# cherise215/advchain

Measured on AMD Instinct MI355X. Metric: augmented images/sec (N adv steps, chain=noise+bias+morph+affine), higher is better.
Workload: dtype f32

## Files before the change

advchain_amd/_lib.py:

```python
import ctypes
import os
from ctypes import c_char_p, c_float, c_int, c_int64, c_void_p

_HERE = os.path.dirname(os.path.abspath(__file__))
LIB_PATH = os.path.join(_HERE, "csrc", "libadvchain_hip.so")

_P, _I, _L, _F = c_void_p, c_int, c_int64, c_float

PROTOTYPES = {
    "advchain_version": (_I, []),
    "advchain_last_error": (c_char_p, []),
    "advchain_set_deterministic": (None, [_I]),
    "advchain_get_deterministic": (_I, []),
    "advchain_grid_sample_fwd": (_I, [_P, _P, _P, _L, _L, _I, _P, _P, _I, _I, _I, _P]),
    "advchain_grid_sample_fwd_ride": (_I, [_P, _P, _P, _P, _P, _L, _L, _I, _P, _P, _I, _I, _I, _I, _P]),
    "advchain_scatter_workspace": (_L, [_L, _I, _P]),
    "advchain_grid_sample_bwd": (_I, [_P, _P, _P, _P, _P, _P, _L, _L, _I, _P, _P, _I, _I, _I, _I, _P]),
    "advchain_compose_self_fwd": (_I, [_P, _P, _P, _L, _I, _P, _I, _P, _P]),
    "advchain_compose_self_bwd": (_I, [_P, _P, _P, _P, _I, _I, _L, _I, _P, _P]),
    "advchain_affine_warp_fwd": (_I, [_P, _P, _P, _L, _L, _I, _P, _I, _I, _P]),
    "advchain_affine_warp_fwd_ride": (_I, [_P, _P, _P, _P, _P, _L, _L, _I, _P, _I, _I, _I, _P]),
    "advchain_affine_warp_bwd_workspace": (_L, [_L, _I, _P]),
    "advchain_affine_warp_bwd": (_I, [_P, _P, _P, _P, _P, _P, _L, _L, _I, _P, _I, _I, _P]),
    "advchain_affine_theta_fwd": (_I, [_P, _P, _F, _P, _P, _L, _I, _P]),
    "advchain_affine_theta_bwd": (_I, [_P, _P, _F, _P, _P, _P, _L, _I, _P]),
    "advchain_tp_interp_fwd": (_I, [_P, _P, _P, _P, _P, _P, _P, _L, _L, _I, _I, _F, _P, _P, _P]),
    "advchain_tp_interp_fwd_smoothed_pair": (_I, [_P, _P, _P, _P, _P, _P, _P, _P, _L, _L, _I, _F, _P, _P, _F, _P]),
    "advchain_band_reduce_axis": (_I, [_P, _P, _P, _P, _P, _P, _P, _P, _I, _L, _L, _F, _P]),
    "advchain_band_reduce_rows_dense": (_I, [_P, _P, _P, _P, _P, _L, _L, _L, _L, _F, _P]),
    "advchain_bias_field_fwd": (_I, [_P, _P, _P, _P, _P, _P, _P, _P, _P, _L, _L, _F, _I, _F, _P]),
    "advchain_bias_field_bwd": (_I, [_P, _P, _P, _P, _P, _P, _P, _P, _P, _P, _L, _L, _F, _I, _F, _P]),
    "advchain_gauss_axis": (_I, [_P, _P, _P, _L, _L, _I, _P, _I, _P, _I, _I, _F, _P]),
    "advchain_gauss_axis_generic": (_I, [_P, _P, _L, _I, _P, _I, _P, _I, _F, _P]),
    "advchain_max_displacement": (_I, [_P, _P, _L, _I, _P, _P]),
    "advchain_grid_sample_bicubic2d_fwd": (_I, [_P, _P, _P, _L, _L, _P, _P, _I, _P]),
    "advchain_grid_sample_bicubic2d_bwd": (_I, [_P, _P, _P, _P, _P, _L, _L, _P, _P, _I, _P]),
    "advchain_affine_grid2d_fwd": (_I, [_P, _P, _L, _P, _P]),
    "advchain_affine_grid2d_bwd_workspace": (_L, [_L, _P]),
    "advchain_affine_grid2d_bwd": (_I, [_P, _P, _P, _L, _P, _P]),
    "advchain_slot_rows_max": (_I, [_P, _P, _L, _L, _I, _P]),
    "advchain_demons_compose_pair_fwd": (_I, [_P, _P, _P, _P, _P, _P, _P, _P, _P, _P, _P, _P, _P, _L, _I, _I, _P, _P, _F, _F, _I, _P]),
    "advchain_demons_compose_pair_bwd": (_I, [_P, _P, _P, _P, _P, _P, _P, _P, _P, _P, _P, _P, _P, _P, _P, _P, _P, _L, _P, _P, _P, _L,
                                              _I, _I, _P, _F, _F, _P]),
    "advchain_bounds_check": (_I, [_P, _P, _P, _L, _P, _P]),
    "advchain_expo_chain_fused_levels": (_I, [_L, _I, _P, _I, _P]),
    "advchain_expo_chain_fwd": (_I, [_P, _P, _P, _L, _I, _P, _I, _P, _P, _P, _P]),
    "advchain_expo_chain_bwd": (_I, [_P, _P, _P, _P, _P, _P, _P, _L, _I, _P, _I, _P]),
    "advchain_gauss_xy": (_I, [_P, _P, _P, _L, _L, _I, _P, _P, _I, _I, _F, _P, _P, _L]),
    "advchain_gauss_small": (_I, [_P, _P, _L, _I, _P, _P, _I, _F, _P]),
    "advchain_gauss_small_pair": (_I, [_P, _P, _L, _I, _P, _P, _F, _I, _P]),
    "advchain_axpy": (_I, [_P, _P, _P, _F, _L, _P]),
    "advchain_sign_axpy": (_I, [_P, _P, _P, _F, _L, _P, _P, _P]),
    "advchain_nonzero_mask": (_I, [_P, _P, _L, _P]),
    "advchain_consistency_finish": (_I, [_P, _P, _P, _P, _I, _P]),
    "advchain_norm_workspace": (_L, [_L, _L]),
    "advchain_norm_axpy": (_I, [_P, _P, _P, _P, _F, _L, _L, _P]),
    "advchain_norm_axpy_gated": (_I, [_P, _P, _P, _P, _F, _L, _L, _P, _P, _P]),
    "advchain_update_multi": (_I, [_P, _I, _P, _P]),
    "advchain_consistency_fwd": (_I, [_P, _P, _P, _P, _P, _P, _P, _L, _L, _I, _P, _I, _I, _I, _I, _P]),
    "advchain_consistency_bwd": (_I, [_P, _P, _P, _P, _P, _P, _F, _F, _F, _F, _I, _L, _L, _I, _P, _I, _P]),
    "advchain_consistency_fused_fwd": (_I, [_P, _P, _P, _P, _P, _L, _L, _I, _P, _I, _I, _I, _I, _P]),
    "advchain_consistency_fused_bwd": (_I, [_P, _P, _P, _P, _P, _P, _F, _F, _F, _F, _I, _L, _L, _I, _P, _I, _P]),
    "advchain_consistency_wide_fwd": (_I, [_P, _P, _P, _P, _P, _P, _L, _L, _I, _P, _I, _I, _I, _I, _P]),
    "advchain_consistency_wide_bwd": (_I, [_P, _P, _P, _P, _P, _P, _P, _F, _F, _F, _F, _I, _L, _L, _I, _P, _I, _P]),
    "advchain_consistency_fused_fwd_bf16": (_I, [_P, _P, _P, _P, _P, _L, _L, _I, _P, _P]),
    "advchain_consistency_fused_bwd_bf16": (_I, [_P, _P, _P, _P, _P, _P, _F, _F, _F, _L, _L, _I, _P, _P]),
# ... 112 lines not shown
```

advchain_amd/csrc/error.cpp:

```cpp
#include <string.h>

#include <atomic>

static thread_local char g_last_error[512] = "";

extern "C" void advchain_set_error_(const char* msg) {
  strncpy(g_last_error, msg ? msg : "", sizeof(g_last_error) - 1);
  g_last_error[sizeof(g_last_error) - 1] = 0;
}

extern "C" const char* advchain_last_error(void) { return g_last_error; }

static std::atomic<int> g_deterministic{0};
extern "C" void advchain_set_deterministic(int on) { g_deterministic.store(on ? 1 : 0, std::memory_order_relaxed); }
extern "C" int advchain_get_deterministic(void) { return g_deterministic.load(std::memory_order_relaxed); }

extern "C" int advchain_version(void) { return 130; }
```

advchain_amd/csrc/sampler_common.h:

```cpp
#pragma once
#include "common.h"

namespace advchain {

template <int DIM, int PAD>
struct Taps {
  AxisTap x, y, z;
  __device__ __forceinline__ void build(float gx, float gy, float gz, const Dims& d) {
    x = make_tap<PAD>(gx, d.s2);
    y = make_tap<PAD>(gy, d.s1);
    if (DIM == 3) z = make_tap<PAD>(gz, d.s0);
    else { z.i0 = 0; z.w0 = 1.f; z.w1 = 0.f; z.mult = 0.f; z.v0 = true; z.v1 = false; }
  }
  __device__ __forceinline__ bool ok(int cz, int cy, int cx) const {
    return (cx ? x.v1 : x.v0) && (cy ? y.v1 : y.v0) && (DIM == 3 ? (cz ? z.v1 : z.v0) : true);
  }
  __device__ __forceinline__ int off(int cz, int cy, int cx, const Dims& d) const {
    return ((z.i0 + cz) * d.s1 + (y.i0 + cy)) * d.s2 + (x.i0 + cx);
  }
  __device__ __forceinline__ float wx(int c) const { return c ? x.w1 : x.w0; }
  __device__ __forceinline__ float wy(int c) const { return c ? y.w1 : y.w0; }
  __device__ __forceinline__ float wz(int c) const { return c ? z.w1 : z.w0; }
  __device__ __forceinline__ float w(int cz, int cy, int cx) const {
    float r = wx(cx) * wy(cy);
// ... 134 lines not shown
  bx = affine_base_coord(ix, d.s2);
  by = affine_base_coord(iy, d.s1);
  if constexpr (DIM == 3) {
    bz = affine_base_coord(iz, d.s0);
    gx = th.m[0][0] * bx + th.m[0][1] * by + th.m[0][2] * bz + th.m[0][3];
    gy = th.m[1][0] * bx + th.m[1][1] * by + th.m[1][2] * bz + th.m[1][3];
    gz = th.m[DIM - 1][0] * bx + th.m[DIM - 1][1] * by + th.m[DIM - 1][2] * bz + th.m[DIM - 1][DIM];
  } else {
    bz = 0.f; gz = 0.f;
    gx = th.m[0][0] * bx + th.m[0][1] * by + th.m[0][2];
    gy = th.m[1][0] * bx + th.m[1][1] * by + th.m[1][2];
  }
}

template <int VEC>
__device__ __forceinline__ void load_vec(const float* __restrict__ p, float (&r)[VEC]) {
  if constexpr (VEC == 4) {
    const float4 q = *reinterpret_cast<const float4*>(p);
    r[0] = q.x; r[1] = q.y; r[2] = q.z; r[3] = q.w;
  } else {
#pragma unroll
    for (int k = 0; k < VEC; ++k) r[k] = p[k];
  }
}
template <int VEC>
__device__ __forceinline__ void store_vec(float* __restrict__ p, const float (&r)[VEC]) {
  if constexpr (VEC == 4) {
    *reinterpret_cast<float4*>(p) = make_float4(r[0], r[1], r[2], r[3]);
  } else {
#pragma unroll
    for (int k = 0; k < VEC; ++k) p[k] = r[k];
  }
}

__device__ __forceinline__ void lds_order() { asm volatile("" ::: "memory"); }

__device__ __forceinline__ float clamp_unit(float v) { return fminf(fmaxf(v, -1.f), 1.f); }

__device__ __forceinline__ float voxel_displacement(float g, int S, int s) {
  const float dv = fabsf(((g + 1.f) * 0.5f) * (float)(S - 1) - (float)s);
  return dv < 1.0e9f ? dv : 1.0e9f;
}

constexpr int kDispSlots = 4096;
__device__ __forceinline__ void wave_max_to_slots(float m, float* __restrict__ slots) {
#pragma unroll
  for (int o = 32; o > 0; o >>= 1) m = fmaxf(m, __shfl_xor(m, o, 64));
  const unsigned blk = (blockIdx.z * gridDim.y + blockIdx.y) * gridDim.x + blockIdx.x;
  float* p = slots + (blk * (blockDim.x >> 6) + (threadIdx.x >> 6)) % kDispSlots;
  if ((threadIdx.x & 63) == __builtin_ffsll(__builtin_amdgcn_ballot_w64(true)) - 1 && m > 0.f)
    atomicMax(reinterpret_cast<unsigned int*>(p), __float_as_uint(m));
}


}
```

advchain_amd/csrc/scatter_tiled.hip:

```cpp
#include <stdlib.h>
#include "sampler_common.h"

namespace advchain {

struct TileCfg {
  int t0, t1, t2;
  int h0, h1, h2;
  int n0, n1, n2;
};

__device__ __forceinline__ bool in_tile_box(int s, int u, int T, int H) {
  const int lo = (u / T) * T;
  return (s >= lo - H) && (s < lo + T + H);
}

__device__ __forceinline__ bool deposit_handled(int sz, int sy, int sx, int uz, int uy, int ux, const TileCfg& tc) {
  return in_tile_box(sx, ux, tc.t2, tc.h2) && in_tile_box(sy, uy, tc.t1, tc.h1) && in_tile_box(sz, uz, tc.t0, tc.h0);
}

constexpr int kFixedBits = 30;

__device__ __forceinline__ void lds_add_fixed(long long* p, float v) {
  const long long q = (long long)__float2int_rn(v);
  atomicAdd(reinterpret_cast<unsigned long long*>(p), (unsigned long long)q);
// ... 317 lines not shown
  }
}

int advchain_scatter_tiled_launch(bool self, const float* gout, const float* in, const float* grid, float* gin,
                                  float* ggrid, int64_t N, int64_t C, int ndim, Dims d, int padding, int clamp_grid,
                                  int32_t* workspace, int chain, int halo, hipStream_t st) {
  if (C < 1 || C > 4) return ADVCHAIN_ERR_UNSUPPORTED;
  const TileCfg tc = choose_tiles(ndim, d, (int)C, halo < 0 ? -halo : halo);
  const int64_t V = d.voxels();
  int* cnt = workspace;
  float* amax = reinterpret_cast<float*>(workspace + 2);
  int2* list = reinterpret_cast<int2*>(workspace + 4);
  const int64_t cap64 = N * V;
  const int cap = cap64 > 0x7fffffff ? 0x7fffffff : (int)cap64;
  hipLaunchKernelGGL(k_scatter_prepare, dim3(1), dim3(1), 0, st, workspace, chain);
  {
    const int64_t total = N * C * V;
    int blocks = (int)((total / 4 + kBlock - 1) / kBlock);
    if (blocks > 1024) blocks = 1024;
    if (blocks < 1) blocks = 1;
    hipLaunchKernelGGL(k_absmax, dim3(blocks), dim3(kBlock), 0, st, gout, total, amax,
                       (int)((reinterpret_cast<uintptr_t>(gout) & 15) == 0), chain ? workspace + 1 : (const int*)nullptr);
  }
  dim3 g((unsigned)(tc.n0 * tc.n1 * tc.n2), (unsigned)N);
  const size_t lds = (size_t)C * tc.t0 * tc.t1 * tc.t2 * sizeof(long long);
  const bool need_ggrid = ggrid != nullptr;
  bool ok;
#define GO(DIM_, PAD_) \
  ok = launch_rows_c<DIM_, PAD_>((int)C, self, need_ggrid, g, lds, st, gout, in, grid, gin, ggrid, d, tc, clamp_grid, amax, amax + 1, cnt, list, cap)
  if (ndim == 3) {
    switch (padding) {
      case PAD_ZEROS: GO(3, PAD_ZEROS); break;
      case PAD_BORDER: GO(3, PAD_BORDER); break;
      default: GO(3, PAD_REFLECTION); break;
    }
  } else {
    switch (padding) {
      case PAD_ZEROS: GO(2, PAD_ZEROS); break;
      case PAD_BORDER: GO(2, PAD_BORDER); break;
      default: GO(2, PAD_REFLECTION); break;
    }
  }
#undef GO
  if (!ok) return ADVCHAIN_ERR_UNSUPPORTED;
  ADVCHAIN_LAUNCH_CHECK();
  return ADVCHAIN_OK;
}

extern "C" int advchain_get_deterministic(void);
extern "C" int64_t advchain_scatter_workspace(int64_t N, int ndim, const int64_t* dims) {
  int64_t V = 1;
  for (int i = 0; i < ndim; ++i) V *= dims[i];
  const int64_t base = 4 + 2 * N * V;
  return advchain_get_deterministic() ? base + 8 * N * V + ((N + 3) & ~(int64_t)3) : base;
}
```

advchain_amd/csrc/scatter_window.hip:

```cpp
#include <stdlib.h>
#include "sampler_common.h"

namespace advchain {

constexpr int kDetBits = 40;
template <bool DET>
__device__ __forceinline__ void win_global_add(float* __restrict__ gin, unsigned long long* __restrict__ acc, int64_t idx,
                                               float v, const FixScale& sdet) {
  if (DET) atomicAdd(acc + idx, (unsigned long long)__float2ll_rn(fix_in(v * sdet.mul, sdet)));
  else atomic_add_f32(gin + idx, v);
}
__device__ __forceinline__ FixScale det_scale(const float* __restrict__ maxn, int n) { return fix_scale(maxn[n], kDetBits); }

__global__ void __launch_bounds__(kBlock) k_det_absmax(const float* __restrict__ x, float* __restrict__ maxn, int64_t per_n) {
  const int n = blockIdx.y;
  const float* p = x + (int64_t)n * per_n;
  float m = 0.f;
  bool bad = false;
  const int64_t stride = (int64_t)gridDim.x * kBlock * 4;
  for (int64_t i = ((int64_t)blockIdx.x * kBlock + threadIdx.x) * 4; i < per_n; i += stride) {
    float v[4];
    if (i + 4 <= per_n && ((uintptr_t)(p + i) & 15) == 0) {
      const float4 q = *reinterpret_cast<const float4*>(p + i);
      v[0] = q.x; v[1] = q.y; v[2] = q.z; v[3] = q.w;
    } else {
#pragma unroll
      for (int j = 0; j < 4; ++j) v[j] = i + j < per_n ? p[i + j] : 0.f;
    }
#pragma unroll
    for (int j = 0; j < 4; ++j) { m = fmaxf(m, fabsf(v[j])); bad = bad || !(fabsf(v[j]) <= 3.0e38f); }
  }
  if (bad) m = __int_as_float(0x7f800000);
#pragma unroll
  for (int o = 32; o > 0; o >>= 1) m = fmaxf(m, __shfl_xor(m, o, 64));
  __shared__ float wm[kBlock / 64];
  if ((threadIdx.x & 63) == 0) wm[threadIdx.x >> 6] = m;
  __syncthreads();
  if (threadIdx.x == 0) {
#pragma unroll
    for (int w = 1; w < kBlock / 64; ++w) m = fmaxf(m, wm[w]);
    atomicMax(reinterpret_cast<int*>(maxn) + n, __float_as_int(m));
  }
}

__global__ void __launch_bounds__(kBlock) k_det_convert(const long long* __restrict__ acc, const float* __restrict__ maxn,
                                                        float* __restrict__ gin, int64_t per_n) {
  const int n = blockIdx.y;
  const FixScale fs = det_scale(maxn, n);
  const long long* a = acc + (int64_t)n * per_n;
  float* g = gin + (int64_t)n * per_n;
  const int64_t stride = (int64_t)gridDim.x * kBlock * 2;
  for (int64_t i = ((int64_t)blockIdx.x * kBlock + threadIdx.x) * 2; i < per_n; i += stride) {
    if (i + 2 <= per_n) {
      const longlong2 q = *reinterpret_cast<const longlong2*>(a + i);
      g[i] = fix_out((float)q.x, fs);
      g[i + 1] = fix_out((float)q.y, fs);
    } else {
      g[i] = fix_out((float)a[i], fs);
    }
  }
}

#ifndef ADVCHAIN_WINDOW_FLAT
#define ADVCHAIN_WINDOW_FLAT 1
#endif
constexpr int kWinT = 32;
constexpr int kWinCells = 8192;
constexpr int kWinCellsC4 = 12288;

template <int PAD, int C, bool SELF, bool GG, bool DET = false>
__global__ void __launch_bounds__(kBlock)
k_scatter_window2d(const float* __restrict__ gout, const float* __restrict__ in, const float* __restrict__ grid,
                   float* __restrict__ gin, float* __restrict__ ggrid, Dims d, int n2, int clamp_grid,
                   int32_t* __restrict__ ws, unsigned long long* __restrict__ acc64 = nullptr,
                   const float* __restrict__ maxn = nullptr) {
  constexpr int kCells2 = C == 4 ? kWinCellsC4 : kWinCells;
  __shared__ int win[kCells2];
  if (ws && blockIdx.x == 0 && blockIdx.y == 0 && threadIdx.x == 0) ws[3] = -1;
  __shared__ int red[8][kBlock / 64];
  constexpr int DIM = 2;
  constexpr int SPT = kWinT * kWinT / kBlock;
  const int V = (int)d.voxels();
  const int n = blockIdx.y;
  const int tx = blockIdx.x % n2, ty = blockIdx.x / n2;
  const int lx = threadIdx.x & 31, ly0 = threadIdx.x >> 5;
  const int sx = tx * kWinT + lx;
  const float* gn = grid + (int64_t)n * DIM * V;
  const float* gon = gout + (int64_t)n * C * V;
  const float* inn = in + (int64_t)n * C * V;
  float* ginn = gin + (int64_t)n * C * V;
  unsigned long long* accn = DET ? acc64 + (int64_t)n * C * V : nullptr;
  const FixScale sdet = DET ? det_scale(maxn, n) : FixScale{0, 0.f, 0.f};

  Taps<DIM, PAD> t[SPT];
  float go[SPT][C];
  bool live[SPT], px[SPT], py[SPT];
  int bx0 = 1 << 30, bx1 = -(1 << 30), by0 = 1 << 30, by1 = -(1 << 30);
  float gmax = 0.f;
#pragma unroll
  for (int j = 0; j < SPT; ++j) {
    const int sy = ty * kWinT + ly0 + 8 * j;
    live[j] = sx < d.s2 && sy < d.s1;
    const int s = live[j] ? sy * d.s2 + sx : 0;
    float gx = gn[s], gy = gn[V + s];
    px[j] = py[j] = true;
    if (clamp_grid) {
      px[j] = gx >= -1.f && gx <= 1.f; py[j] = gy >= -1.f && gy <= 1.f;
      gx = clamp_unit(gx); gy = clamp_unit(gy);
    }
    t[j].build(gx, gy, 0.f, d);
#pragma unroll
    for (int c = 0; c < C; ++c) {
      const float g = gon[(int64_t)c * V + s];
      go[j][c] = live[j] ? g : 0.f;
      gmax = fmaxf(gmax, fabsf(go[j][c]));
    }
    if (live[j]) {
      if (t[j].x.v0 || t[j].x.v1) { bx0 = min(bx0, t[j].x.i0 + (t[j].x.v0 ? 0 : 1)); bx1 = max(bx1, t[j].x.i0 + (t[j].x.v1 ? 1 : 0)); }
      if (t[j].y.v0 || t[j].y.v1) { by0 = min(by0, t[j].y.i0 + (t[j].y.v0 ? 0 : 1)); by1 = max(by1, t[j].y.i0 + (t[j].y.v1 ? 1 : 0)); }
    }
  }
#pragma unroll
  for (int o = 32; o > 0; o >>= 1) {
    bx0 = min(bx0, __shfl_xor(bx0, o, 64)); bx1 = max(bx1, __shfl_xor(bx1, o, 64));
    by0 = min(by0, __shfl_xor(by0, o, 64)); by1 = max(by1, __shfl_xor(by1, o, 64));
    gmax = fmaxf(gmax, __shfl_xor(gmax, o, 64));
  }
  const int wave = threadIdx.x >> 6;
  if ((threadIdx.x & 63) == 0) {
    red[0][wave] = bx0; red[1][wave] = bx1; red[2][wave] = by0; red[3][wave] = by1; red[4][wave] = __float_as_int(gmax);
  }
  __syncthreads();
#pragma unroll
  for (int w = 0; w < kBlock / 64; ++w) {
    bx0 = min(bx0, red[0][w]); bx1 = max(bx1, red[1][w]); by0 = min(by0, red[2][w]); by1 = max(by1, red[3][w]);
    gmax = fmaxf(gmax, __int_as_float(red[4][w]));
  }
  int ww = max(bx1 - bx0 + 1, 0), wh = max(by1 - by0 + 1, 0);
  constexpr int cells_per_ch = kCells2 / C;
  if (ww > 128) ww = 128;
  if (ww > 0 && wh > cells_per_ch / ww) wh = cells_per_ch / ww;
  const int cells = ww * wh;
  for (int i = threadIdx.x; i < C * cells; i += kBlock) win[i] = 0;
  const FixScale fs = fix_scale(gmax, 20);
  __syncthreads();

  float cgx[SPT], cgy[SPT];
  if (SELF || GG) {
#pragma unroll
    for (int j = 0; j < SPT; ++j) {
      float ax = 0.f, ay = 0.f, dummy = 0.f;
#pragma unroll
      for (int c = 0; c < C; ++c)
        sample_linear_bwd<DIM, PAD, false, true>(inn + (int64_t)c * V, nullptr, go[j][c], t[j], d, ax, ay, dummy);
      cgx[j] = px[j] ? t[j].x.mult * ax : 0.f;
      cgy[j] = py[j] ? t[j].y.mult * ay : 0.f;
    }
  }

#pragma unroll
  for (int j = 0; j < SPT; ++j) {
    if (!live[j]) continue;
    const int sy = ty * kWinT + ly0 + 8 * j;
    const int s = sy * d.s2 + sx;
    const int wx0 = t[j].x.i0 - bx0, wy0 = t[j].y.i0 - by0;
    const int cell0 = __mul24(wy0, ww) + wx0;
    const int vox0 = __mul24(t[j].y.i0, d.s2) + t[j].x.i0;
    const bool inx[2] = {wx0 >= 0 && wx0 < ww, wx0 + 1 >= 0 && wx0 + 1 < ww};
    const bool iny[2] = {wy0 >= 0 && wy0 < wh, wy0 + 1 >= 0 && wy0 + 1 < wh};
#pragma unroll
    for (int cy = 0; cy < 2; ++cy)
#pragma unroll
      for (int cx = 0; cx < 2; ++cx) {
        if (!t[j].ok(0, cy, cx)) continue;
        const float w = t[j].w(0, cy, cx);
        if (inx[cx] && iny[cy]) {
          const float ws = w * fs.mul;
          int* cell = win + cell0 + (cy ? ww : 0) + cx;
#pragma unroll
          for (int c = 0; c < C; ++c) atomicAdd(cell + c * cells, fix_round(ws * fix_in(go[j][c], fs)));
        } else {
          const int64_t dst = vox0 + (cy ? d.s2 : 0) + cx;
#pragma unroll
          for (int c = 0; c < C; ++c) win_global_add<DET>(ginn, accn, dst + (int64_t)c * V, w * go[j][c], sdet);
        }
      }
    if (SELF || GG) {
      const float ggx = cgx[j], ggy = cgy[j];
      if (SELF) {
        if (ggx != 0.f) win_global_add<DET>(ginn, accn, s, ggx, sdet);
        if (ggy != 0.f) win_global_add<DET>(ginn, accn, (int64_t)V + s, ggy, sdet);
      } else {
        float* gg = ggrid + (int64_t)n * DIM * V + s;
        gg[0] = ggx;
        gg[V] = ggy;
      }
    }
  }
  __syncthreads();

  for (int i = threadIdx.x; i < C * cells; i += kBlock) {
    const int a = win[i];
    if (a == 0) continue;
    const int c = i / cells, r = i - c * cells;
    const int wy = r / ww, wx = r - wy * ww;
    win_global_add<DET>(ginn, accn, (int64_t)c * V + (by0 + wy) * d.s2 + (bx0 + wx), fix_out((float)a, fs), sdet);
  }
}

#ifndef ADVCHAIN_WIN3_CP4
#define ADVCHAIN_WIN3_CP4 2
#endif
#ifndef ADVCHAIN_WIN3_CPS
#define ADVCHAIN_WIN3_CPS 3
#endif
constexpr int kWin3CP4 = ADVCHAIN_WIN3_CP4, kWin3CPS = ADVCHAIN_WIN3_CPS;
constexpr int kWin3Cells = 12288;

template <int PAD, int C, bool SELF, bool GG, int TX, int TZ, bool DET = false>
__global__ void __launch_bounds__(kBlock)
k_scatter_window3d(const float* __restrict__ gout, const float* __restrict__ in, const float* __restrict__ grid,
                   float* __restrict__ gin, float* __restrict__ ggrid, Dims d, int n1, int n2, int clamp_grid,
                   int32_t* __restrict__ ws, unsigned long long* __restrict__ acc64 = nullptr,
                   const float* __restrict__ maxn = nullptr) {
  __shared__ int win[kWin3Cells];
  constexpr int CP = C == 4 ? kWin3CP4 : (SELF ? kWin3CPS : C);
  if (ws && blockIdx.x == 0 && blockIdx.y == 0 && threadIdx.x == 0) ws[3] = -1;
  __shared__ int red[7][kBlock / 64];
  constexpr int DIM = 3;
  const int V = (int)d.voxels();
  const int n = blockIdx.y;
  int b = blockIdx.x;
  const int tx = b % n2; b /= n2;
  const int ty = b % n1, tz = b / n1;
  constexpr int kWin3X = TX, kWin3Y = kBlock / TX, kWin3Z = TZ;
  const int sx = tx * kWin3X + (threadIdx.x % TX), sy = ty * kWin3Y + (threadIdx.x / TX);
  const bool col_live = sx < d.s2 && sy < d.s1;
  const float* gn = grid + (int64_t)n * DIM * V;
  const float* gon = gout + (int64_t)n * C * V;
  const float* inn = in + (int64_t)n * C * V;
  float* ginn = gin + (int64_t)n * C * V;
  unsigned long long* accn = DET ? acc64 + (int64_t)n * C * V : nullptr;
  const FixScale sdet = DET ? det_scale(maxn, n) : FixScale{0, 0.f, 0.f};

  int lo[3] = {1 << 30, 1 << 30, 1 << 30}, hi[3] = {-(1 << 30), -(1 << 30), -(1 << 30)};
  float gmax = 0.f;
#pragma unroll
  for (int j = 0; j < kWin3Z; ++j) {
    const int sz = tz * kWin3Z + j;
    const bool live = col_live && sz < d.s0;
    const int s = live ? (sz * d.s1 + sy) * d.s2 + sx : 0;
    float g[3] = {gn[s], gn[V + s], gn[2 * V + s]};
    if (clamp_grid) { g[0] = clamp_unit(g[0]); g[1] = clamp_unit(g[1]); g[2] = clamp_unit(g[2]); }
    Taps<DIM, PAD> t;
    t.build(g[0], g[1], g[2], d);
#pragma unroll
    for (int c = 0; c < C; ++c) gmax = fmaxf(gmax, live ? fabsf(gon[(int64_t)c * V + s]) : 0.f);
    if (live) {
      const AxisTap* ax[3] = {&t.x, &t.y, &t.z};
// ... 122 lines not shown
          if (inx[cx] && iny[cy] && inz[cz]) {
            const float ws = w * fs.mul;
            int* cell = win + cell0 + (cz ? plane : 0) + (cy ? ww : 0) + cx;
#pragma unroll
            for (int c = 0; c < CP; ++c) atomicAdd(cell + c * cells, fix_round(ws * fix_in(go[c0 + c], fs)));
          } else {
            const int64_t dst = vox0 + (cz ? planev : 0) + (cy ? rowv : 0) + cx + (int64_t)c0 * V;
#pragma unroll
            for (int c = 0; c < CP; ++c) win_global_add<DET>(ginn, accn, dst + (int64_t)c * V, w * go[c0 + c], sdet);
          }
        }
#endif
    if ((SELF || GG) && c0 == 0) {
      float ax = 0.f, ay = 0.f, az = 0.f;
#pragma unroll
      for (int c = 0; c < C; ++c) sample_linear_bwd_values<DIM, PAD>(cv[c], go[c], t, ax, ay, az);
      const float ggx = pass[0] ? t.x.mult * ax : 0.f, ggy = pass[1] ? t.y.mult * ay : 0.f,
                  ggz = pass[2] ? t.z.mult * az : 0.f;
      if (SELF) {
        if (ggx != 0.f) win_global_add<DET>(ginn, accn, s, ggx, sdet);
        if (ggy != 0.f) win_global_add<DET>(ginn, accn, (int64_t)V + s, ggy, sdet);
        if (ggz != 0.f) win_global_add<DET>(ginn, accn, 2 * (int64_t)V + s, ggz, sdet);
      } else {
        float* gg = ggrid + (int64_t)n * DIM * V + s;
        gg[0] = ggx;
        gg[V] = ggy;
        gg[2 * (int64_t)V] = ggz;
      }
    }
  }
  __syncthreads();

  {
    const float inv_ww = 1.f / (float)max(ww, 1), inv_wh = 1.f / (float)max(wh, 1), inv_wd = 1.f / (float)max(wd, 1);
    for (int i = threadIdx.x; i < CP * cells; i += kBlock) {
      const int a = win[i];
      if (a == 0) continue;
      const int r = (int)(((float)i + 0.5f) * inv_ww), wx = i - r * ww;
      const int rz = (int)(((float)r + 0.5f) * inv_wh), wy = r - rz * wh;
      const int c = (int)(((float)rz + 0.5f) * inv_wd), wz = rz - c * wd;
      win_global_add<DET>(ginn, accn, (int64_t)(c0 + c) * V + ((lo[2] + wz) * d.s1 + (lo[1] + wy)) * d.s2 + (lo[0] + wx),
                          fix_out((float)a, fs), sdet);
    }
  }
  if (c0 + CP < C) __syncthreads();
  }
}

}

using namespace advchain;

extern "C" int advchain_get_deterministic(void);
int advchain_scatter_window_launch(bool self, const float* gout, const float* in, const float* grid, float* gin,
                                   float* ggrid, int64_t N, int64_t C, int ndim, Dims d, int padding, int clamp_grid,
                                   int halo, int32_t* workspace, hipStream_t st, int32_t* det_ws) {
  static const bool off = getenv("ADVCHAIN_NO_WINDOW_SCATTER") != nullptr;
  static const int min3 = 2;
  if (off || padding == PAD_REFLECTION) return ADVCHAIN_ERR_UNSUPPORTED;
  if (d.s2 >= (1 << 23) || (int64_t)d.s0 * d.s1 >= (1 << 23)) return ADVCHAIN_ERR_UNSUPPORTED;
  if (self ? C != ndim : (C != 1 && C != 2 && C != 4)) return ADVCHAIN_ERR_UNSUPPORTED;
  if (ndim == 3 && (halo < 0 ? -halo : halo) < min3) return ADVCHAIN_ERR_UNSUPPORTED;
  const bool det = advchain_get_deterministic() != 0 && det_ws != nullptr;
  const int64_t V = d.voxels();
  unsigned long long* acc64 = nullptr;
  float* maxn = nullptr;
  if (det) {
    acc64 = reinterpret_cast<unsigned long long*>(det_ws + 4 + 2 * N * V);
    maxn = reinterpret_cast<float*>(det_ws + 4 + 2 * N * V + 8 * N * V);
    advchain_zero_async(acc64, sizeof(unsigned long long) * N * C * V, st);
    advchain_zero_async(maxn, sizeof(float) * N, st);
    const int64_t per_n = C * V;
    int64_t nb = (per_n + kBlock * 16 - 1) / (kBlock * 16);
    if (nb > 1024) nb = 1024;
    hipLaunchKernelGGL(k_det_absmax, dim3((unsigned)nb, (unsigned)N), dim3(kBlock), 0, st, gout, maxn, per_n);
  } else {
    advchain_zero_async(gin, sizeof(float) * N * C * V, st);
  }
  const bool gg = ggrid != nullptr;
  dim3 b(kBlock);
#define GO_PAD(C_, SELF_, GG_) \
  do { if (padding == PAD_BORDER) GO(PAD_BORDER, C_, SELF_, GG_); else GO(PAD_ZEROS, C_, SELF_, GG_); } while (0)
#define GO_ALL(CS_) \
  do { \
    if (self) GO(PAD_BORDER, CS_, true, false); \
    else if (C == 1) { if (gg) GO_PAD(1, false, true); else GO_PAD(1, false, false); } \
    else if (C == 2) { if (gg) GO_PAD(2, false, true); else GO_PAD(2, false, false); } \
    else { if (gg) GO_PAD(4, false, true); else GO_PAD(4, false, false); } \
  } while (0)
  if (ndim == 2) {
    const int n2 = (d.s2 + kWinT - 1) / kWinT, n1 = (d.s1 + kWinT - 1) / kWinT;
    dim3 g((unsigned)(n1 * n2), (unsigned)N);
#define GO(PAD_, C_, SELF_, GG_) \
  do { \
    if (det) hipLaunchKernelGGL((k_scatter_window2d<PAD_, C_, SELF_, GG_, true>), g, b, 0, st, gout, in, grid, gin, ggrid, d, n2, clamp_grid, workspace, acc64, maxn); \
    else hipLaunchKernelGGL((k_scatter_window2d<PAD_, C_, SELF_, GG_, false>), g, b, 0, st, gout, in, grid, gin, ggrid, d, n2, clamp_grid, workspace, acc64, maxn); \
  } while (0)
    GO_ALL(2);
#undef GO
  } else {
    static const int shape = getenv("ADVCHAIN_WIN3_SHAPE") ? atoi(getenv("ADVCHAIN_WIN3_SHAPE")) : -1;
    const int sh = shape >= 0 ? (shape != 0) : ((d.s2 % 32 != 0 && d.s2 % 16 == 0) ? 1 : 0);
    const int TXs = sh == 0 ? 32 : 16, TYs = kBlock / TXs, TZs = 4;
    const int n2 = (d.s2 + TXs - 1) / TXs, n1 = (d.s1 + TYs - 1) / TYs, n0 = (d.s0 + TZs - 1) / TZs;
    dim3 g((unsigned)(n0 * n1 * n2), (unsigned)N);
#define GO3(PAD_, C_, SELF_, GG_, TX_, DET_) \
  hipLaunchKernelGGL((k_scatter_window3d<PAD_, C_, SELF_, GG_, TX_, 4, DET_>), g, b, 0, st, gout, in, grid, gin, ggrid, d, n1, n2, clamp_grid, workspace, acc64, maxn)
#define GO(PAD_, C_, SELF_, GG_) \
  do { \
    if (sh == 0) { if (det) GO3(PAD_, C_, SELF_, GG_, 32, true); else GO3(PAD_, C_, SELF_, GG_, 32, false); } \
    else { if (det) GO3(PAD_, C_, SELF_, GG_, 16, true); else GO3(PAD_, C_, SELF_, GG_, 16, false); } \
  } while (0)
    GO_ALL(3);
#undef GO
#undef GO3
  }
#undef GO_ALL
#undef GO_PAD
  if (det) {
    const int64_t per_n = C * V;
    int64_t nb = (per_n + kBlock * 8 - 1) / (kBlock * 8);
    if (nb > 2048) nb = 2048;
    hipLaunchKernelGGL(k_det_convert, dim3((unsigned)nb, (unsigned)N), dim3(kBlock), 0, st, reinterpret_cast<const long long*>(acc64),
                       maxn, gin, per_n);
  }
  ADVCHAIN_LAUNCH_CHECK();
  return ADVCHAIN_OK;
}
```

advchain_amd/ops.py:

```python
import ctypes
import functools
import os

import numpy as np
import torch

from . import _lib
from .bands import gaussian_weights_1d

_INTERP = {"bilinear": 0, "trilinear": 0, "linear": 0, "nearest": 1, "bicubic": 2}
_PAD = {"zeros": 0, "border": 1, "reflection": 2}
_GAUSS9 = _lib.float_array(gaussian_weights_1d(1.0))
_GAUSS9_CACHE = {}


GENERIC_MAX_TAPS = 129


def gauss9(sigma, taps=None):
    sigma = float(sigma)
    if taps is None:
        taps = 2 * int(4 * sigma + 0.5) + 1
    taps = int(taps)
    if sigma == 1.0 and taps == 9:
# ... 95 lines not shown
        return 0
    return min(int(disp) + 1, 255) << 8


def _fine_bits(disp):
    if disp is None or not disp == disp or disp < 0:
        return 0
    return max(1, min(int(disp * 1024.0) + 1, (1 << 22) - 1))


def raw_grid_sample_fwd(inp, grid, interp, padding, clamp_grid, disp_hint=None):
    N, C = inp.shape[:2]
    nd = inp.dim() - 2
    odims = grid.shape[2:]
    out = torch.empty((N, C) + tuple(odims), device=inp.device, dtype=torch.float32)
    _lib.check(_lib.load().advchain_grid_sample_fwd(_ptr(inp), _ptr(grid), _ptr(out), N, C, nd,
                                                    _lib.dims_array(inp.shape[2:]), _lib.dims_array(odims),
                                                    interp, padding, int(clamp_grid) | _hint_bits(disp_hint), _stream()),
               "grid_sample_fwd")
    return out


def raw_grid_sample_fwd_ride(inp, grid, ride, interp, padding, clamp_grid, nonzero, disp_hint=None):
    N, C = inp.shape[:2]
    nd = inp.dim() - 2
    odims = tuple(grid.shape[2:])
    out = torch.empty((N, C) + odims, device=inp.device, dtype=torch.float32)
    rout = torch.empty((N, 1) + odims, device=inp.device, dtype=torch.float32)
    _lib.check(_lib.load().advchain_grid_sample_fwd_ride(_ptr(inp), _ptr(grid), _ptr(out), _ptr(ride), _ptr(rout), N, C, nd,
                                                         _lib.dims_array(inp.shape[2:]), _lib.dims_array(odims), interp, padding,
                                                         int(clamp_grid) | _hint_bits(disp_hint), int(bool(nonzero)), _stream()),
               "grid_sample_fwd_ride")
    return out, rout


DISP_SLOTS = 4096
ADAPTIVE_HALO = os.environ.get("ADVCHAIN_NO_ADAPTIVE_HALO") is None
PAIR_FIELDS = os.environ.get("ADVCHAIN_NO_PAIR_FIELDS") is None
TILED_SCATTER = True
FUSED_LOSS = True
WIDE_LOSS_MIN_K = 17
FUSE_2D = True
COMPOSITE = True
RIDE_MASK = True
RIDE_INTERPS = ("bilinear", "trilinear", "linear", "nearest")


def set_deterministic(on):
    _lib.load().advchain_set_deterministic(1 if on else 0)


def is_deterministic():
    return bool(_lib.load().advchain_get_deterministic())


def _scatter_workspace(N, dims, device):
    n = _lib.load().advchain_scatter_workspace(N, len(dims), _lib.dims_array(dims))
    return torch.empty(n, device=device, dtype=torch.int32)


def raw_grid_sample_bwd(gout, inp, grid, interp, padding, clamp_grid, need_gin, need_ggrid, halo=0):
    N, C = inp.shape[:2]
    nd = inp.dim() - 2
    tiled = TILED_SCATTER and need_gin
    ws = _scatter_workspace(N, inp.shape[2:], inp.device) if tiled else None
    gin = (torch.empty_like(inp) if tiled else torch.zeros_like(inp)) if need_gin else None
    ggrid = torch.empty_like(grid) if need_ggrid else None
    _lib.check(_lib.load().advchain_grid_sample_bwd(_ptr(gout), _ptr(inp), _ptr(grid), _ptr(gin), _ptr(ggrid), _ptr(ws),
                                                    N, C, nd, _lib.dims_array(inp.shape[2:]),
                                                    _lib.dims_array(grid.shape[2:]), interp, padding, int(clamp_grid),
                                                    int(halo), _stream()), "grid_sample_bwd")
    return gin, ggrid


def raw_compose_self_fwd(phi, phi0=None, final_mode=0, disp_out=None, disp_hint=None):
    N = phi.shape[0]
    nd = phi.dim() - 2
    out = torch.empty_like(phi)
    _lib.check(_lib.load().advchain_compose_self_fwd(_ptr(phi), _ptr(out), _ptr(phi0), N, nd,
                                                     _lib.dims_array(phi.shape[2:]), final_mode | _hint_bits(disp_hint), _ptr(disp_out),
                                                     _stream()), "compose_self_fwd")
    return out


def raw_compose_self_bwd(gout, phi, ws=None, chain=False, halo=0):
    N = phi.shape[0]
    nd = phi.dim() - 2
    if TILED_SCATTER and ws is None:
        ws, chain = _scatter_workspace(N, phi.shape[2:], phi.device), False
    gphi = torch.empty_like(phi) if ws is not None else torch.zeros_like(phi)
    _lib.check(_lib.load().advchain_compose_self_bwd(_ptr(gout), _ptr(phi), _ptr(gphi), _ptr(ws), int(bool(chain)), int(halo), N, nd,
                                                     _lib.dims_array(phi.shape[2:]), _stream()), "compose_self_bwd")
    return gphi


def raw_max_displacement(phi, out=None):
    if out is None:
        out = torch.zeros(1, device=phi.device, dtype=torch.float32)
    _lib.check(_lib.load().advchain_max_displacement(_ptr(phi), _ptr(out), phi.shape[0], phi.dim() - 2,
                                                     _lib.dims_array(phi.shape[2:]), _stream()), "max_displacement")
    return out


def raw_slot_rows_max(slots, reset=False, out=None):
    if out is None:
        out = torch.empty(slots.shape[0], device=slots.device, dtype=torch.float32)
# ... 1547 lines not shown
```

include/advchain_hip.h:

```cpp
#ifndef ADVCHAIN_HIP_H_
#define ADVCHAIN_HIP_H_

#include <stdint.h>

#ifdef __cplusplus
extern "C" {
#endif

#define ADVCHAIN_INTERP_LINEAR 0
#define ADVCHAIN_INTERP_NEAREST 1
#define ADVCHAIN_INTERP_BICUBIC 2
#define ADVCHAIN_PAD_ZEROS 0
#define ADVCHAIN_PAD_BORDER 1
#define ADVCHAIN_PAD_REFLECTION 2

int advchain_version(void);
const char* advchain_last_error(void);

void advchain_set_deterministic(int on);
int advchain_get_deterministic(void);

int advchain_grid_sample_fwd(const float* in, const float* grid, float* out, int64_t N, int64_t C, int ndim,
                             const int64_t* in_dims, const int64_t* out_dims, int interp, int padding,
                             int clamp_grid, void* stream);
int advchain_grid_sample_fwd_ride(const float* in, const float* grid, float* out, const float* ride_in, float* ride_out,
                                  int64_t N, int64_t C, int ndim, const int64_t* in_dims, const int64_t* out_dims,
                                  int interp, int padding, int clamp_grid, int flags, void* stream);
int64_t advchain_scatter_workspace(int64_t N, int ndim, const int64_t* dims);
int advchain_grid_sample_bwd(const float* grad_out, const float* in, const float* grid, float* grad_in,
                             float* grad_grid, int32_t* workspace, int64_t N, int64_t C, int ndim,
                             const int64_t* in_dims, const int64_t* out_dims, int interp, int padding, int clamp_grid,
                             int halo, void* stream);

#define ADVCHAIN_DISP_SLOTS 4096
int advchain_compose_self_fwd(const float* phi, float* out, const float* phi0, int64_t N, int ndim,
                              const int64_t* dims, int final_mode, float* disp_out, void* stream);
int advchain_compose_self_bwd(const float* grad_out, const float* phi, float* grad_phi, int32_t* workspace, int chain,
                              int halo, int64_t N, int ndim, const int64_t* dims, void* stream);
int advchain_expo_chain_fused_levels(int64_t N, int ndim, const int64_t* dims, int n, const int32_t* hints);
int advchain_expo_chain_fwd(const float* phi0, float* fields, float* pos, int64_t N, int ndim, const int64_t* dims, int n,
                            float* disp_rows, const int32_t* hints, float* fuse_flag, void* stream);
int advchain_expo_chain_bwd(const float* grad_pos, const float* phi0, const float* fields, float* grad_phi0, float* scratch,
                            int32_t* workspace, const int32_t* halos, int64_t N, int ndim, const int64_t* dims, int n,
                            void* stream);
int advchain_demons_compose_pair_fwd(const float* vel, float* s1, float* phi0, float* fields, float* pos, float* q,
                                     float* disp, float* rows_max, const int32_t* itab, const float* ftab,
                                     const int64_t* S3, const int64_t* g3, const int64_t* B3, int64_t N, int ndim, int n,
                                     const int32_t* hints, const float* weights9_host, float scale, float inv, int fuse,
                                     void* stream);
int advchain_demons_compose_pair_bwd(const float* gq_lo, const float* gq_hi, const float* pos, const float* phi0,
                                     const float* fields, float* gpos, float* g, float* scratch, int32_t* ws, float* t1,
                                     float* gs1, float* gvel, const int32_t* halos, const int32_t* itab, const float* ftab,
                                     const float* wd, const int32_t* wlo, int64_t WB, const int64_t* S3, const int64_t* g3,
                                     const int64_t* B3, int64_t N, int ndim, int n, const float* weights9_host, float scale,
                                     float inv, void* stream);
int advchain_max_displacement(const float* phi, float* out, int64_t N, int ndim, const int64_t* dims, void* stream);
int advchain_slot_rows_max(float* slots, float* out, int64_t rows, int64_t cols, int reset, void* stream);
int advchain_bounds_check(const float* values, const float* lo, const float* hi, int64_t n, int32_t* flag, void* stream);

int advchain_affine_warp_fwd(const float* in, const float* theta, float* out, int64_t N, int64_t C, int ndim,
                             const int64_t* dims, int interp, int padding, void* stream);
int advchain_affine_warp_fwd_ride(const float* in, const float* theta, float* out, const float* ride_in, float* ride_out,
                                  int64_t N, int64_t C, int ndim, const int64_t* dims, int interp, int padding, int flags,
                                  void* stream);
int64_t advchain_affine_warp_bwd_workspace(int64_t N, int ndim, const int64_t* dims);
int advchain_affine_warp_bwd(const float* grad_out, const float* in, const float* theta, float* grad_in,
                             float* grad_theta, float* workspace, int64_t N, int64_t C, int ndim,
                             const int64_t* dims, int interp, int padding, void* stream);

int advchain_grid_sample_bicubic2d_fwd(const float* in, const float* grid, float* out, int64_t N, int64_t C,
                                       const int64_t* in_dims, const int64_t* out_dims, int padding, void* stream);
int advchain_grid_sample_bicubic2d_bwd(const float* grad_out, const float* in, const float* grid, float* grad_in,
                                       float* grad_grid, int64_t N, int64_t C, const int64_t* in_dims,
// ... 128 lines not shown
```

Before: 4243.

## Stage deterministic 2D window scatter into per-tile slots and gather without global atomics

In deterministic mode for 2D grids, each scatter tile writes its fixed-point shared-memory window and metadata into a per-tile slot instead of doing int64 global atomics. A new gather kernel then has each output tile collect the overlapping windows, rescale them to a global fixed-point scale and write gin directly. This is meant to remove the large int64 accumulator zeroing, the global atomic traffic and the convert pass. If any window overflows its slot, a gated fallback rerun uses the original atomic path. The cost is a larger workspace, extra kernel launches, and a gather cost that grows with the number of tiles.

After: 4164. 1.9% lower.

```diff
diff --git a/advchain_amd/_lib.py b/advchain_amd/_lib.py
--- a/advchain_amd/_lib.py
+++ b/advchain_amd/_lib.py
@@ -12,6 +12,9 @@
     "advchain_last_error": (c_char_p, []),
     "advchain_set_deterministic": (None, [_I]),
     "advchain_get_deterministic": (_I, []),
+    "advchain_set_window_staging": (None, [_I]),
+    "advchain_get_window_staging": (_I, []),
+    "advchain_window_spill_offset": (_L, [_L, _I, _P]),
     "advchain_grid_sample_fwd": (_I, [_P, _P, _P, _L, _L, _I, _P, _P, _I, _I, _I, _P]),
     "advchain_grid_sample_fwd_ride": (_I, [_P, _P, _P, _P, _P, _L, _L, _I, _P, _P, _I, _I, _I, _I, _P]),
     "advchain_scatter_workspace": (_L, [_L, _I, _P]),
diff --git a/advchain_amd/csrc/error.cpp b/advchain_amd/csrc/error.cpp
--- a/advchain_amd/csrc/error.cpp
+++ b/advchain_amd/csrc/error.cpp
@@ -14,5 +14,8 @@
 static std::atomic<int> g_deterministic{0};
 extern "C" void advchain_set_deterministic(int on) { g_deterministic.store(on ? 1 : 0, std::memory_order_relaxed); }
 extern "C" int advchain_get_deterministic(void) { return g_deterministic.load(std::memory_order_relaxed); }
+static std::atomic<int> g_window_staging{1};
+extern "C" void advchain_set_window_staging(int on) { g_window_staging.store(on ? 1 : 0, std::memory_order_relaxed); }
+extern "C" int advchain_get_window_staging(void) { return g_window_staging.load(std::memory_order_relaxed); }
 
 extern "C" int advchain_version(void) { return 130; }
diff --git a/advchain_amd/csrc/sampler_common.h b/advchain_amd/csrc/sampler_common.h
--- a/advchain_amd/csrc/sampler_common.h
+++ b/advchain_amd/csrc/sampler_common.h
@@ -210,5 +210,20 @@
     atomicMax(reinterpret_cast<unsigned int*>(p), __float_as_uint(m));
 }
 
-
-}
+constexpr int kWinSlot = 12288;
+constexpr int kWinRec = 8;
+struct WinStageLayout {
+  int64_t tiles, slots, maxn, spill, recs, total;
+};
+static inline WinStageLayout win_stage_layout(int64_t N, int64_t s1, int64_t s2) {
+  WinStageLayout l;
+  l.tiles = ((s1 + 31) / 32) * ((s2 + 31) / 32);
+  l.slots = 4 + 2 * N * s1 * s2;
+  l.maxn = l.slots + N * l.tiles * kWinSlot;
+  l.spill = l.maxn + ((N + 3) & ~(int64_t)3);
+  l.recs = l.spill + 4;
+  l.total = l.recs + N * l.tiles * kWinRec;
+  return l;
+}
+
+}
diff --git a/advchain_amd/csrc/scatter_tiled.hip b/advchain_amd/csrc/scatter_tiled.hip
--- a/advchain_amd/csrc/scatter_tiled.hip
+++ b/advchain_amd/csrc/scatter_tiled.hip
@@ -393,5 +393,12 @@
   int64_t V = 1;
   for (int i = 0; i < ndim; ++i) V *= dims[i];
   const int64_t base = 4 + 2 * N * V;
-  return advchain_get_deterministic() ? base + 8 * N * V + ((N + 3) & ~(int64_t)3) : base;
-}
+  if (!advchain_get_deterministic()) return base;
+  if (ndim == 2) return win_stage_layout(N, dims[0], dims[1]).total;
+  return base + 8 * N * V + ((N + 3) & ~(int64_t)3);
+}
+
+extern "C" int64_t advchain_window_spill_offset(int64_t N, int ndim, const int64_t* dims) {
+  if (!advchain_get_deterministic() || ndim != 2) return -1;
+  return win_stage_layout(N, dims[0], dims[1]).spill;
+}
diff --git a/advchain_amd/csrc/scatter_window.hip b/advchain_amd/csrc/scatter_window.hip
--- a/advchain_amd/csrc/scatter_window.hip
+++ b/advchain_amd/csrc/scatter_window.hip
@@ -44,7 +44,9 @@
 }
 
 __global__ void __launch_bounds__(kBlock) k_det_convert(const long long* __restrict__ acc, const float* __restrict__ maxn,
-                                                        float* __restrict__ gin, int64_t per_n) {
+                                                        float* __restrict__ gin, int64_t per_n,
+                                                        const int32_t* __restrict__ gate = nullptr) {
+  if (gate && *gate == 0) return;
   const int n = blockIdx.y;
   const FixScale fs = det_scale(maxn, n);
   const long long* a = acc + (int64_t)n * per_n;
@@ -61,6 +63,13 @@
   }
 }
 
+__global__ void __launch_bounds__(kBlock) k_det_clear_gated(unsigned long long* __restrict__ p, int64_t n,
+                                                            const int32_t* __restrict__ gate) {
+  if (*gate == 0) return;
+  for (int64_t i = (int64_t)blockIdx.x * kBlock + threadIdx.x; i < n; i += (int64_t)gridDim.x * kBlock) p[i] = 0ull;
+}
+__global__ void k_win_stage_prepare(int32_t* __restrict__ spill) { *spill = 0; }
+
 #ifndef ADVCHAIN_WINDOW_FLAT
 #define ADVCHAIN_WINDOW_FLAT 1
 #endif
@@ -68,13 +77,22 @@
 constexpr int kWinCells = 8192;
 constexpr int kWinCellsC4 = 12288;
 
-template <int PAD, int C, bool SELF, bool GG, bool DET = false>
+struct WinStage {
+  int32_t* slots;
+  int32_t* recs;
+  int32_t* spill;
+};
+template <int PAD, int C, bool SELF, bool GG, bool DET = false, bool STAGED = false>
 __global__ void __launch_bounds__(kBlock)
 k_scatter_window2d(const float* __restrict__ gout, const float* __restrict__ in, const float* __restrict__ grid,
                    float* __restrict__ gin, float* __restrict__ ggrid, Dims d, int n2, int clamp_grid,
                    int32_t* __restrict__ ws, unsigned long long* __restrict__ acc64 = nullptr,
-                   const float* __restrict__ maxn = nullptr) {
+                   const float* __restrict__ maxn = nullptr, const int32_t* __restrict__ gate = nullptr,
+                   WinStage sg = WinStage{nullptr, nullptr, nullptr}) {
+  static_assert(!(DET && STAGED), "STAGED replaces the int64 image");
   constexpr int kCells2 = C == 4 ? kWinCellsC4 : kWinCells;
+  static_assert(kCells2 <= kWinSlot && (!SELF || kWinCells + 2 * kWinT * kWinT <= kWinSlot), "slot size");
+  if (DET && gate && *gate == 0) return;
   __shared__ int win[kCells2];
   if (ws && blockIdx.x == 0 && blockIdx.y == 0 && threadIdx.x == 0) ws[3] = -1;
   __shared__ int red[8][kBlock / 64];
@@ -97,6 +115,7 @@
   bool live[SPT], px[SPT], py[SPT];
   int bx0 = 1 << 30, bx1 = -(1 << 30), by0 = 1 << 30, by1 = -(1 << 30);
   float gmax = 0.f;
+  bool bad = false;
 #pragma unroll
   for (int j = 0; j < SPT; ++j) {
     const int sy = ty * kWinT + ly0 + 8 * j;
@@ -114,6 +133,7 @@
       const float g = gon[(int64_t)c * V + s];
       go[j][c] = live[j] ? g : 0.f;
       gmax = fmaxf(gmax, fabsf(go[j][c]));
+      if (STAGED) bad = bad || !(fabsf(go[j][c]) <= 3.0e38f);
     }
     if (live[j]) {
       if (t[j].x.v0 || t[j].x.v1) { bx0 = min(bx0, t[j].x.i0 + (t[j].x.v0 ? 0 : 1)); bx1 = max(bx1, t[j].x.i0 + (t[j].x.v1 ? 1 : 0)); }
@@ -127,6 +147,7 @@
     gmax = fmaxf(gmax, __shfl_xor(gmax, o, 64));
   }
   const int wave = threadIdx.x >> 6;
+  if (STAGED) bad = __syncthreads_or(bad) != 0;
   if ((threadIdx.x & 63) == 0) {
     red[0][wave] = bx0; red[1][wave] = bx1; red[2][wave] = by0; red[3][wave] = by1; red[4][wave] = __float_as_int(gmax);
   }
@@ -138,9 +159,24 @@
   }
   int ww = max(bx1 - bx0 + 1, 0), wh = max(by1 - by0 + 1, 0);
   constexpr int cells_per_ch = kCells2 / C;
+  const bool spilled = STAGED && (ww > 128 || (ww > 0 && wh > cells_per_ch / min(ww, 128)));
   if (ww > 128) ww = 128;
   if (ww > 0 && wh > cells_per_ch / ww) wh = cells_per_ch / ww;
   const int cells = ww * wh;
+  int32_t* slot = nullptr;
+  if (STAGED) {
+    const int64_t tile = (int64_t)n * gridDim.x + blockIdx.x;
+    slot = sg.slots + tile * kWinSlot;
+    if (threadIdx.x == 0) {
+      int32_t* rec = sg.recs + tile * kWinRec;
+      rec[0] = bx0; rec[1] = by0; rec[2] = spilled ? 0 : ww; rec[3] = spilled ? 0 : wh;
+      rec[4] = __float_as_int(gmax);
+      rec[5] = bad ? 0x7f800000 : __float_as_int(gmax);
+      rec[6] = spilled ? 1 : 0; rec[7] = 0;
+      if (spilled) *sg.spill = 1;
+    }
+    if (spilled) return;
+  }
   for (int i = threadIdx.x; i < C * cells; i += kBlock) win[i] = 0;
   const FixScale fs = fix_scale(gmax, 20);
   __syncthreads();
@@ -155,6 +191,15 @@
         sample_linear_bwd<DIM, PAD, false, true>(inn + (int64_t)c * V, nullptr, go[j][c], t[j], d, ax, ay, dummy);
       cgx[j] = px[j] ? t[j].x.mult * ax : 0.f;
       cgy[j] = py[j] ? t[j].y.mult * ay : 0.f;
+    }
+  }
+
+  if (STAGED && SELF) {
+    float* cg = reinterpret_cast<float*>(slot + kWinCells);
+#pragma unroll
+    for (int j = 0; j < SPT; ++j) {
+      cg[j * kBlock + threadIdx.x] = live[j] ? cgx[j] : 0.f;
+      cg[(SPT + j) * kBlock + threadIdx.x] = live[j] ? cgy[j] : 0.f;
     }
   }
 
@@ -179,7 +224,7 @@
           int* cell = win + cell0 + (cy ? ww : 0) + cx;
 #pragma unroll
           for (int c = 0; c < C; ++c) atomicAdd(cell + c * cells, fix_round(ws * fix_in(go[j][c], fs)));
-        } else {
+        } else if (!STAGED) {
           const int64_t dst = vox0 + (cy ? d.s2 : 0) + cx;
 #pragma unroll
           for (int c = 0; c < C; ++c) win_global_add<DET>(ginn, accn, dst + (int64_t)c * V, w * go[j][c], sdet);
@@ -188,8 +233,10 @@
     if (SELF || GG) {
       const float ggx = cgx[j], ggy = cgy[j];
       if (SELF) {
-        if (ggx != 0.f) win_global_add<DET>(ginn, accn, s, ggx, sdet);
-        if (ggy != 0.f) win_global_add<DET>(ginn, accn, (int64_t)V + s, ggy, sdet);
+        if (!STAGED) {
+          if (ggx != 0.f) win_global_add<DET>(ginn, accn, s, ggx, sdet);
+          if (ggy != 0.f) win_global_add<DET>(ginn, accn, (int64_t)V + s, ggy, sdet);
+        }
       } else {
         float* gg = ggrid + (int64_t)n * DIM * V + s;
         gg[0] = ggx;
@@ -199,12 +246,117 @@
   }
   __syncthreads();
 
+  if (STAGED) {
+    for (int i = threadIdx.x; i < C * cells; i += kBlock) slot[i] = win[i];
+    return;
+  }
   for (int i = threadIdx.x; i < C * cells; i += kBlock) {
     const int a = win[i];
     if (a == 0) continue;
     const int c = i / cells, r = i - c * cells;
     const int wy = r / ww, wx = r - wy * ww;
     win_global_add<DET>(ginn, accn, (int64_t)c * V + (by0 + wy) * d.s2 + (bx0 + wx), fix_out((float)a, fs), sdet);
+  }
+}
+
+
+template <int C, bool SELF>
+__global__ void __launch_bounds__(kBlock)
+k_window_gather2d(const int32_t* __restrict__ slots, const int32_t* __restrict__ recs, float* __restrict__ maxn,
+                  float* __restrict__ gin, Dims d, int n2) {
+  __shared__ float wm[kBlock / 64];
+  __shared__ int l_n;
+  __shared__ int l_rec[kBlock], l_bx0[kBlock], l_by0[kBlock], l_ww[kBlock], l_wh[kBlock], l_shift[kBlock];
+  __shared__ float l_inv[kBlock];
+  const int T = gridDim.x, n = blockIdx.y;
+  const int tx = blockIdx.x % n2, ty = blockIdx.x / n2;
+  const int lx = threadIdx.x & 31, ly0 = threadIdx.x >> 5;
+  const int x = tx * kWinT + lx;
+  const int V = (int)d.voxels();
+  const int32_t* rn = recs + (int64_t)n * T * kWinRec;
+  const int32_t* sn = slots + (int64_t)n * T * kWinSlot;
+
+  float m = 0.f;
+  for (int r = threadIdx.x; r < T; r += kBlock) m = fmaxf(m, __int_as_float(rn[r * kWinRec + 5]));
+#pragma unroll
+  for (int o = 32; o > 0; o >>= 1) m = fmaxf(m, __shfl_xor(m, o, 64));
+  if ((threadIdx.x & 63) == 0) wm[threadIdx.x >> 6] = m;
+  if (threadIdx.x == 0) l_n = 0;
+  __syncthreads();
+#pragma unroll
+  for (int w = 0; w < kBlock / 64; ++w) m = fmaxf(m, wm[w]);
+  if (blockIdx.x == 0 && threadIdx.x == 0) maxn[n] = m;
+  const FixScale sdet = fix_scale(m, kDetBits);
+
+  unsigned long long acc[4][C];
+#pragma unroll
+  for (int j = 0; j < 4; ++j)
+#pragma unroll
+    for (int c = 0; c < C; ++c) acc[j][c] = 0ull;
+
+  const int X0 = tx * kWinT, Y0 = ty * kWinT;
+  for (int base = 0; base < T; base += kBlock) {
+    const int r = base + threadIdx.x;
+    if (r < T) {
+      const int bx0 = rn[r * kWinRec + 0], by0 = rn[r * kWinRec + 1], ww = rn[r * kWinRec + 2], wh = rn[r * kWinRec + 3];
+      if (ww > 0 && wh > 0 && bx0 < X0 + kWinT && bx0 + ww > X0 && by0 < Y0 + kWinT && by0 + wh > Y0) {
+        const FixScale fs = fix_scale(__int_as_float(rn[r * kWinRec + 4]), 20);
+        const int k = atomicAdd(&l_n, 1);
+        l_rec[k] = r; l_bx0[k] = bx0; l_by0[k] = by0; l_ww[k] = ww; l_wh[k] = wh; l_shift[k] = fs.shift; l_inv[k] = fs.inv;
+      }
+    }
+    __syncthreads();
+    const int cnt = l_n;
+    for (int k = 0; k < cnt; ++k) {
+      const int ww = l_ww[k], wh = l_wh[k];
+      const int cells = ww * wh;
+      const int32_t* slot = sn + (int64_t)l_rec[k] * kWinSlot;
+      const FixScale fs{l_shift[k], 0.f, l_inv[k]};
+      const int wx = x - l_bx0[k];
+      const int wy0 = Y0 + ly0 - l_by0[k];
+      const bool inx = wx >= 0 && wx < ww;
+      int a[4][C];
+      bool in[4];
+#pragma unroll
+      for (int j = 0; j < 4; ++j) {
+        const int wy = wy0 + 8 * j;
+        in[j] = inx && wy >= 0 && wy < wh;
+        const int idx = in[j] ? wy * ww + wx : 0;
+#pragma unroll
+        for (int c = 0; c < C; ++c) a[j][c] = slot[c * cells + idx];
+      }
+#pragma unroll
+      for (int j = 0; j < 4; ++j)
+#pragma unroll
+        for (int c = 0; c < C; ++c)
+          if (in[j] && a[j][c] != 0)
+            acc[j][c] += (unsigned long long)__float2ll_rn(fix_in(fix_out((float)a[j][c], fs) * sdet.mul, sdet));
+    }
+    __syncthreads();
+    if (threadIdx.x == 0) l_n = 0;
+    __syncthreads();
+  }
+
+  if (SELF) {
+    if (rn[blockIdx.x * kWinRec + 6] == 0) {
+      const float* cg = reinterpret_cast<const float*>(sn + (int64_t)blockIdx.x * kWinSlot + kWinCells);
+#pragma unroll
+      for (int j = 0; j < 4; ++j) {
+        const float ggx = cg[j * kBlock + threadIdx.x], ggy = cg[(4 + j) * kBlock + threadIdx.x];
+        if (ggx != 0.f) acc[j][0] += (unsigned long long)__float2ll_rn(fix_in(ggx * sdet.mul, sdet));
+        if (ggy != 0.f) acc[j][C - 1] += (unsigned long long)__float2ll_rn(fix_in(ggy * sdet.mul, sdet));
+      }
+    }
+  }
+
+  float* ginn = gin + (int64_t)n * C * V;
+#pragma unroll
+  for (int j = 0; j < 4; ++j) {
+    const int y = Y0 + ly0 + 8 * j;
+    if (x < d.s2 && y < d.s1) {
+#pragma unroll
+      for (int c = 0; c < C; ++c) ginn[(int64_t)c * V + y * d.s2 + x] = fix_out((float)(long long)acc[j][c], sdet);
+    }
   }
 }
 
@@ -433,6 +585,7 @@
 using namespace advchain;
 
 extern "C" int advchain_get_deterministic(void);
+extern "C" int advchain_get_window_staging(void);
 int advchain_scatter_window_launch(bool self, const float* gout, const float* in, const float* grid, float* gin,
                                    float* ggrid, int64_t N, int64_t C, int ndim, Dims d, int padding, int clamp_grid,
                                    int halo, int32_t* workspace, hipStream_t st, int32_t* det_ws) {
@@ -446,9 +599,22 @@
   const int64_t V = d.voxels();
   unsigned long long* acc64 = nullptr;
   float* maxn = nullptr;
+  const bool staged = det && ndim == 2 && advchain_get_window_staging() != 0;
+  WinStage sg{nullptr, nullptr, nullptr};
+  const int32_t* gate = nullptr;
   if (det) {
     acc64 = reinterpret_cast<unsigned long long*>(det_ws + 4 + 2 * N * V);
     maxn = reinterpret_cast<float*>(det_ws + 4 + 2 * N * V + 8 * N * V);
+    if (ndim == 2) {
+      const WinStageLayout l = win_stage_layout(N, d.s1, d.s2);
+      maxn = reinterpret_cast<float*>(det_ws + l.maxn);
+      sg = WinStage{det_ws + l.slots, det_ws + l.recs, det_ws + l.spill};
+    }
+  }
+  if (staged) {
+    gate = sg.spill;
+    hipLaunchKernelGGL(k_win_stage_prepare, dim3(1), dim3(1), 0, st, sg.spill);
+  } else if (det) {
     advchain_zero_async(acc64, sizeof(unsigned long long) * N * C * V, st);
     advchain_zero_async(maxn, sizeof(float) * N, st);
     const int64_t per_n = C * V;
@@ -474,8 +640,15 @@
     dim3 g((unsigned)(n1 * n2), (unsigned)N);
 #define GO(PAD_, C_, SELF_, GG_) \
   do { \
-    if (det) hipLaunchKernelGGL((k_scatter_window2d<PAD_, C_, SELF_, GG_, true>), g, b, 0, st, gout, in, grid, gin, ggrid, d, n2, clamp_grid, workspace, acc64, maxn); \
-    else hipLaunchKernelGGL((k_scatter_window2d<PAD_, C_, SELF_, GG_, false>), g, b, 0, st, gout, in, grid, gin, ggrid, d, n2, clamp_grid, workspace, acc64, maxn); \
+    if (staged) { \
+      hipLaunchKernelGGL((k_scatter_window2d<PAD_, C_, SELF_, GG_, false, true>), g, b, 0, st, gout, in, grid, gin, ggrid, d, n2, clamp_grid, workspace, acc64, maxn, gate, sg); \
+      hipLaunchKernelGGL((k_window_gather2d<C_, SELF_>), g, b, 0, st, sg.slots, sg.recs, maxn, gin, d, n2); \
+      int64_t nz = (N * C_ * V + 1023) / 1024; \
+      if (nz > 4096) nz = 4096; \
+      hipLaunchKernelGGL(k_det_clear_gated, dim3((unsigned)nz), b, 0, st, acc64, N * C_ * V, gate); \
+    } \
+    if (det) hipLaunchKernelGGL((k_scatter_window2d<PAD_, C_, SELF_, GG_, true>), g, b, 0, st, gout, in, grid, gin, ggrid, d, n2, clamp_grid, workspace, acc64, maxn, gate, sg); \
+    else hipLaunchKernelGGL((k_scatter_window2d<PAD_, C_, SELF_, GG_, false>), g, b, 0, st, gout, in, grid, gin, ggrid, d, n2, clamp_grid, workspace, acc64, maxn, gate, sg); \
   } while (0)
     GO_ALL(2);
 #undef GO
@@ -503,7 +676,7 @@
     int64_t nb = (per_n + kBlock * 8 - 1) / (kBlock * 8);
     if (nb > 2048) nb = 2048;
     hipLaunchKernelGGL(k_det_convert, dim3((unsigned)nb, (unsigned)N), dim3(kBlock), 0, st, reinterpret_cast<const long long*>(acc64),
-                       maxn, gin, per_n);
+                       maxn, gin, per_n, gate);
   }
   ADVCHAIN_LAUNCH_CHECK();
   return ADVCHAIN_OK;
diff --git a/advchain_amd/ops.py b/advchain_amd/ops.py
--- a/advchain_amd/ops.py
+++ b/advchain_amd/ops.py
@@ -171,6 +171,18 @@
 
 def is_deterministic():
     return bool(_lib.load().advchain_get_deterministic())
+
+
+def set_window_staging(on):
+    _lib.load().advchain_set_window_staging(1 if on else 0)
+
+
+def is_window_staging():
+    return bool(_lib.load().advchain_get_window_staging())
+
+
+def window_spill_offset(N, dims):
+    return int(_lib.load().advchain_window_spill_offset(N, len(dims), _lib.dims_array(dims)))
 
 
 def _scatter_workspace(N, dims, device):
diff --git a/include/advchain_hip.h b/include/advchain_hip.h
--- a/include/advchain_hip.h
+++ b/include/advchain_hip.h
@@ -19,6 +19,9 @@
 
 void advchain_set_deterministic(int on);
 int advchain_get_deterministic(void);
+void advchain_set_window_staging(int on);
+int advchain_get_window_staging(void);
+int64_t advchain_window_spill_offset(int64_t N, int ndim, const int64_t* dims);
 
 int advchain_grid_sample_fwd(const float* in, const float* grid, float* out, int64_t N, int64_t C, int ndim,
                              const int64_t* in_dims, const int64_t* out_dims, int interp, int padding,
```
